# wangqiaoli/geometric_mapping

Hardware: AMD Instinct MI355X
Metric: points/sec full segment+fit, 1M-pt synthetic tunnel frame (higher is better)
Workload: dtype f32; 1 GPU; 1000000-pt synthetic tunnel frame (R=2 m, L=12 m, sigma=0.01), rows resident in HBM; k_regime=fixed-k (~256 neighbours), mode=frames, frames_in_flight=3, GPU_MAX_HW_QUEUES=4, ransac_model=cylinder, H=1024, tau=0.03 (extension), parallelism=framesx1

## Files before the change

### geometric_mapping_amd/csrc/gm_device.hpp

```cpp
#pragma once

#include <hip/hip_runtime.h>
#include <stdint.h>

#include "../../include/gm_hip.h"

namespace gm {

constexpr int kWave = 64;

struct ScanState {
    unsigned long long *status;
    uint32_t *ticket;
    uint32_t epoch;
    const uint32_t *frame_ptr;
};

__device__ __forceinline__ uint32_t scan_epoch(const ScanState &st)
{
    return st.frame_ptr ? 0x20000000u + (((*st.frame_ptr) * 32u + st.epoch) & 0x1FFFFFFFu) : st.epoch;
}

#ifndef GM_TILE_CLASSES
#define GM_TILE_CLASSES 8
#endif
constexpr int kTileListClasses = GM_TILE_CLASSES;

struct DevCounters {
    uint32_t n_cropped;
    uint32_t n_valid;
    uint32_t n_tiles;
    uint32_t first_drop_enc;
    uint32_t n_voxels;
    uint32_t vox_n;
    uint32_t mm[6];
    uint32_t scratch_total;
    uint32_t pad[5];
    uint32_t n_tiles_c[kTileListClasses][32];
};
static_assert(sizeof(DevCounters) % 8 == 0, "zero-filled in 8-byte words");

struct VoxelParams {
    float inv_leaf;
    int32_t min_b[3];
    int32_t div_b[3];
    int32_t mul1, mul2;
    uint32_t passthrough;
};

struct GridParams {
    float ox, oy, oz;
    float inv_h;
    float inv_hx;
    int32_t nx, ny, nz;
    int32_t xreach;
    float r2;
    float r2_scale;
    float snap;
    int32_t D;
    int16_t reach[5][5];
    float dscale;
    float dband;
    float band;
};

struct VoxCell {
    unsigned long long sx, sy, sz;
    uint32_t cnt, pad;
};
struct VoxDense {
    uint32_t enabled;
    int32_t i_lo;
    int32_t dim;
    float inv_leaf;
    float lo;
    float own_lo, own_hi;
    double scale, inv_scale;
    uint32_t xcd_chunk;
    uint32_t pad_;
};

struct FrameExt {
    float plane[4];
    float cylinder[7];
    uint32_t plane_inliers, cylinder_inliers;
    uint32_t pad;
    double plane_refit[4];
    double cyl_axis_refit[3];
};

struct CylFitWork {
    double c[3], d[3], r;
    double d_hyp[3];
    double last_step;
    uint32_t status, passes;
};

struct FrameOut {
    DevCounters ctr;
    float evals[3];
    float evecs[9];
    double scatter[6];
    VoxelParams vox;
    FrameExt ext;
    gm_cylinder_fit fit;
};


__device__ __forceinline__ int lane_id() { return threadIdx.x & (kWave - 1); }

__device__ __forceinline__ uint64_t lanemask_lt()
{
    return (1ull << lane_id()) - 1ull;
}
// ... 285 lines not shown
```

### geometric_mapping_amd/csrc/k_normals.hip

```cpp
#include <stdlib.h>
#include <string.h>

#include "gm_internal.hpp"

namespace gm {

typedef float v2f __attribute__((ext_vector_type(2)));

__device__ __forceinline__ v2f pk_mul_rn(v2f a, v2f b)
{
    v2f r;
    r.x = __fmul_rn(a.x, b.x);
    r.y = __fmul_rn(a.y, b.y);
    return r;
}
__device__ __forceinline__ v2f pk_add_rn(v2f a, v2f b)
{
    v2f r;
    r.x = __fadd_rn(a.x, b.x);
    r.y = __fadd_rn(a.y, b.y);
    return r;
}

__device__ __forceinline__ v2f pk_within(v2f d2, v2f neg_big, v2f r2_big)
// ... 809 lines not shown
                    split3(uxa * uxa, uxb * uxb, 10); split3(uxa * uya, uxb * uyb, 13); split3(uxa * uza, uxb * uzb, 16);
                    split3(uya * uya, uyb * uyb, 19); split3(uya * uza, uyb * uzb, 22); split3(uza * uza, uzb * uzb, 25);
                }
            }
            wave_lds_fence();
            if (c0 + clen < row_end(r)) seek(r, c0 + clen); else seek(r + 1, r + 1 < 9 ? row_begin(r + 1) : 0u);
#pragma unroll
            for (int gi = 0; gi < kMxGroups; ++gi) {
                if (gi >= ngroups) break;
                const uint32_t mb = __builtin_amdgcn_readlane(sb, r * kMxGroups + gi),
                               me = __builtin_amdgcn_readlane(se, r * kMxGroups + gi);
                uint32_t ob = mb > c0 ? mb - c0 : 0u, oe = me > c0 ? me - c0 : 0u;
                if (ob > clen) ob = clen;
                if (oe > clen) oe = clen;
                ob &= ~7u;
                const int steps = oe > ob ? (int)((oe - ob + 15u) >> 4) : 0;
#if defined(GM_NORMALS_STATS) && !defined(GM_MD_DEBUG)
                if (lane == 0) {
                    atomicAdd(&ctr->pad[0], (uint32_t)(steps * 16) / 2u);
                    atomicAdd(&ctr->pad[1], (oe > ob ? oe - ob : 0u) * 2u);
                    if (gi == 0) { atomicAdd(&ctr->pad[2], clen); atomicAdd(&ctr->pad[3], 1u); }
                }
#endif
                const float gqa = __shfl(q.x, gi * kMxGroupLanes + qsel, kWave), gqb = __shfl(q.y, gi * kMxGroupLanes + qsel, kWave),
                            gqc = __shfl(q.z, gi * kMxGroupLanes + qsel, kWave);
                const v2f qx = {gqa, gqa}, qy = {gqb, gqb}, qz = {gqc, gqc};
                const float *pw = wx + ob + 8u * (uint32_t)half;
                const uint32_t *fa = feat + ((ob >> 3) + (uint32_t)half) * (uint32_t)kMxOctetWords + (uint32_t)qsel * 4u;
                constexpr int W = kMxChunk + kMxPad;
                auto ld4 = [](const float *q4) { return *reinterpret_cast<const float4 *>(q4); };
                float4 x0 = ld4(pw), x1 = ld4(pw + 4), y0 = ld4(pw + W), y1 = ld4(pw + W + 4), z0 = ld4(pw + 2 * W),
                       z1 = ld4(pw + 2 * W + 4);
                for (int it = 0; it < steps; ++it) {
                    const bf16x8 a = *reinterpret_cast<const bf16x8 *>(fa);
                    const v2f dx0 = (v2f){x0.x, x0.y} - qx, dx1 = (v2f){x0.z, x0.w} - qx, dx2 = (v2f){x1.x, x1.y} - qx, dx3 = (v2f){x1.z, x1.w} - qx;
                    const v2f dy0 = (v2f){y0.x, y0.y} - qy, dy1 = (v2f){y0.z, y0.w} - qy, dy2 = (v2f){y1.x, y1.y} - qy, dy3 = (v2f){y1.z, y1.w} - qy;
                    const v2f dz0 = (v2f){z0.x, z0.y} - qz, dz1 = (v2f){z0.z, z0.w} - qz, dz2 = (v2f){z1.x, z1.y} - qz, dz3 = (v2f){z1.z, z1.w} - qz;
                    pw += 16; fa += 2 * kMxOctetWords;
                    x0 = ld4(pw); x1 = ld4(pw + 4); y0 = ld4(pw + W); y1 = ld4(pw + W + 4); z0 = ld4(pw + 2 * W); z1 = ld4(pw + 2 * W + 4);
                    __builtin_amdgcn_sched_barrier(0);
                    auto within2 = [&](const v2f dx, const v2f dy, const v2f dz) -> uint32_t {
                        const v2f d2 = pk_add_rn(pk_add_rn(pk_mul_rn(dx, dx), pk_mul_rn(dy, dy)), pk_mul_rn(dz, dz));
                        const v2f wgt = pk_within(d2, neg_big, r2_big);
                        return pack_hi16(__float_as_uint(wgt.y), __float_as_uint(wgt.x));
                    };
                    union { bf16x8 v; uint32_t u[4]; } b;
                    b.u[0] = within2(dx0, dy0, dz0);
                    b.u[1] = within2(dx1, dy1, dz1);
                    b.u[2] = within2(dx2, dy2, dz2);
                    b.u[3] = within2(dx3, dy3, dz3);
                    acc[gi] = __builtin_amdgcn_mfma_f32_32x32x16_bf16(a, b.v, acc[gi], 0, 0, 0);
                }
            }
        }
        float own[16], got[16];
#pragma unroll
        for (int k = 0; k < 16; ++k) {
            own[k] = half ? acc[1][k] : acc[0][k];
            const float snd = half ? acc[0][k] : acc[1][k];
            got[k] = __shfl_xor(snd, 32, kWave);
        }
        auto frow = [&](int rr) -> double {
            const int k = 4 * (rr >> 3) + (rr & 3), hh = (rr >> 2) & 1;
            return (double)((hh == half) ? own[k] : got[k]);
        };
        double mom[10];
        mom[0] = frow(0);
#pragma unroll
        for (int m = 0; m < 9; ++m) mom[1 + m] = (frow(1 + 3 * m) + frow(2 + 3 * m)) + frow(3 + 3 * m);

        const bool vox_ok = emit_normal(active, q, mom, vd, normals4, counts, qn, stat_t0);
        if (vd.enabled) voxel_sums(vox_ok, q, vd, vox_table);
    }
}

typedef short s4 __attribute__((ext_vector_type(4)));
#ifndef GM_MDCHUNK
#define GM_MDCHUNK 128
#endif
constexpr int kMdChunk = GM_MDCHUNK;
constexpr int kMdSlots = kMdChunk + 24;
constexpr int kMdOctets = kMdSlots / 8;
constexpr int kMdOctetWords = 33 * 4;
constexpr int kMdWaveLdsBytes = (kMdOctets * kMdOctetWords + 16) * 4;

constexpr int kRowX[3] = {1, 4, 8}, kRowY[3] = {2, 5, 9}, kRowZ[3] = {3, 6, 10}, kRowQ[3] = {11, 7, 12};
constexpr int kRowProd0 = 13;
__device__ __forceinline__ uint32_t md_window_of_base(int b)
{
    return b < 3 ? 0u : ((b == 3 || b == 8) ? 4u : (b == 9 ? 8u : (b == 10 ? 12u : 0u)));
}
__device__ __forceinline__ void md_split3(float a, uint32_t out[3])
{
    const uint32_t ah = __float_as_uint(a) & 0xFFFF0000u;
    const float ra = a - __uint_as_float(ah);
    const uint32_t am = __float_as_uint(ra) & 0xFFFF0000u;
    const float sa = ra - __uint_as_float(am);
    out[0] = ah >> 16; out[1] = am >> 16; out[2] = __float_as_uint(sa) >> 16;
}
__device__ __forceinline__ s4 md_tr_read(const unsigned char *p)
{
    return __builtin_amdgcn_ds_read_tr16_b64_v4i16((__attribute__((address_space(3))) s4 *)p);
}

#ifndef GM_NORMALS_PREFETCH
#define GM_NORMALS_PREFETCH 1
#endif
#ifdef GM_NORMALS_TIMELINE
__device__ unsigned long long gm_tl_buf[3 * 65536];
#endif
#ifdef GM_NORMALS_PHASES
__device__ unsigned long long gm_phase_ticks[16];
#define GM_PH_STAMP(var) const unsigned long long var = __builtin_amdgcn_s_memtime()
#define GM_PH_ADD(slot, expr) do { ph_acc[slot] += (uint32_t)(expr); } while (0)
#else
#define GM_PH_STAMP(var) do {} while (0)
#define GM_PH_ADD(slot, expr) do {} while (0)
#endif

template <bool FINE>
__device__ __forceinline__ void normals_tile_mxd(const NormalsArgs &A, unsigned char *lds, const uint2 tile, uint32_t min_candidates,
                                                 unsigned long long stat_entry = 0ull)
{
    const float4 *__restrict__ spts4 = A.spts4;
    const uint32_t *__restrict__ skeys = A.skeys;
    DevCounters *__restrict__ ctr = A.ctr;
    const GridParams &g = A.g;
    const uint2 *__restrict__ row_bounds = A.row_bounds;
    float4 *__restrict__ normals4 = A.normals4;
    int32_t *__restrict__ counts = A.counts;
    const VoxDense &vd = A.vd;
    VoxCell *__restrict__ vox_table = A.vox_table;
    (void)ctr;
    uint32_t *feat = reinterpret_cast<uint32_t *>(lds);
    int lane = lane_id();
    asm volatile("" : "+v"(lane));
    const uint32_t n = ctr->n_cropped;
    const int qsel = lane & 31, half = lane >> 5;
    const int tq = (lane & 15) >> 2, tp = lane & 3, tr0 = 16 * ((lane >> 4) & 1);
    const uint32_t tr_off = md_window_of_base(8 * half + tq) * 16u +
                            (uint32_t)((tr0 + 4 * tp) >> 3) * (uint32_t)(kMdOctetWords * 4) + (uint32_t)((tr0 + 4 * tp) & 7) * 2u;
    const uint32_t mom_off = (uint32_t)qsel * 16u + 8u * (uint32_t)half;
    {
        const uint32_t qs = tile.x, qn = tile.y & 0xFFu, tile_row = tile.y >> 8;
#ifdef GM_NORMALS_TIMELINE
        const unsigned long long stat_t0 = wall_clock64();
#else
        const unsigned long long stat_t0 = 0ull;
#endif
#ifdef GM_NORMALS_PHASES
        uint32_t ph_acc[8] = {0, 0, 0, 0, 0, 0, 0, 0};
#endif
        GM_PH_STAMP(ph_t0);
        const bool active = (uint32_t)lane < qn;
        const uint32_t qidx = qs + (active ? (uint32_t)lane : qn - 1u);
        const float4 q = spts4[qidx];
        const uint32_t kl = skeys[qidx];
        const uint32_t row = tile_row;
        const int cy = (int)(row % (uint32_t)g.ny), cz = (int)(row / (uint32_t)g.ny);
        const int gD = FINE ? g.D : 1;
        const int side = 2 * gD + 1, nrows_all = side * side;
        int nrows = 0;
        struct LaneRow { int gg, reach; uint32_t nrow; bool ok; uint2 rb; };
        auto lane_row = [&](int row0) -> LaneRow {
            nrows = nrows_all - row0 < 32 ? nrows_all - row0 : 32;
            const int k = FINE ? lane : (lane >> 1);
            const int r = row0 + (k >> 1);
            const int a = (r % side) - gD, b = (r / side) - gD;
            const int yy = cy + a, zz = cz + b;
            LaneRow R;
            R.gg = k & 1;
            R.reach = (k >> 1) < nrows ? (FINE ? (int)g.reach[a < 0 ? -a : a][b < 0 ? -b : b] : g.xreach) : 0;
            R.ok = R.reach > 0 && yy >= 0 && yy < g.ny && zz >= 0 && zz < g.nz;
            R.nrow = R.ok ? (uint32_t)(zz * g.ny + yy) : 0u;
            R.rb = R.ok ? row_bounds[R.nrow] : make_uint2(0u, 0u);
            return R;
        };
        const LaneRow lr0 = lane_row(0);
        const int fxl = (int)(kl - row * (uint32_t)g.nx);
        if (__ballot(active && q.x >= vd.own_lo && q.x < vd.own_hi) == 0) {
            if (active) {
                const float nanv = __builtin_nanf("");
                normals4[__float_as_uint(q.w)] = make_float4(nanv, nanv, nanv, nanv);
                if (counts) counts[__float_as_uint(q.w)] = 0;
            }
            return;
        }
        uint32_t sb = 0, se = 0;
        auto win_begin = [&](int r, int gg) -> uint32_t {
            return FINE ? __builtin_amdgcn_readlane(sb, r * kMxGroups + gg) : __builtin_amdgcn_readlane(sb, 2 * (r * kMxGroups + gg));
        };
        auto win_end = [&](int r, int gg) -> uint32_t {
            return FINE ? __builtin_amdgcn_readlane(se, r * kMxGroups + gg) : __builtin_amdgcn_readlane(sb, 2 * (r * kMxGroups + gg) + 1);
        };
        auto find_windows = [&](const LaneRow &R) {
            sb = 0; se = 0;
            const int gg = R.gg, reach = R.reach;
            const int lo_fx = __shfl(fxl, gg * kMxGroupLanes, kWave);
            const int hi_fx = __shfl(fxl, gg * kMxGroupLanes + kMxGroupLanes - 1, kWave);
            uint32_t key_b = 0, key_e = 0, lo1 = 0, hi1 = 0, row_key0 = 0;
            if (R.ok) {
                const uint32_t rbk = R.nrow * (uint32_t)g.nx;
                const int xa = lo_fx > reach ? lo_fx - reach : 0;
                const int xb = hi_fx + reach < g.nx - 1 ? hi_fx + reach : g.nx - 1;
                key_b = rbk + (uint32_t)xa; key_e = rbk + (uint32_t)xb + 1u;
                lo1 = R.rb.x; hi1 = R.rb.y; row_key0 = rbk;
            }
            if (FINE) {
                uint32_t lo2 = lo1, hi2 = hi1;
                while (lo1 < hi1 || lo2 < hi2) {
                    const uint32_t m1 = (lo1 + hi1) >> 1, m2 = (lo2 + hi2) >> 1;
                    const uint32_t k1 = skeys[m1 < n ? m1 : n - 1u], k2 = skeys[m2 < n ? m2 : n - 1u];
                    if (lo1 < hi1) { if (k1 < key_b) lo1 = m1 + 1u; else hi1 = m1; }
                    if (lo2 < hi2) { if (k2 < key_e) lo2 = m2 + 1u; else hi2 = m2; }
                }
                sb = lo1; se = lo2;
            } else {
                const uint32_t key = (lane & 1) ? key_e : key_b;
#ifndef GM_NORMALS_NO_GUIDED_PROBE
                constexpr uint32_t kGuide = 64;
                if (hi1 - lo1 > 8u * kGuide) {
                    const uint32_t xq = key - row_key0;
                    const uint32_t gpos = lo1 + (uint32_t)((float)xq * (float)(hi1 - lo1) / (float)g.nx);
                    const uint32_t pa0 = gpos > lo1 + kGuide ? gpos - kGuide : lo1;
                    const uint32_t pb0 = gpos + kGuide < hi1 ? gpos + kGuide : hi1 - 1u;
                    const uint32_t ka0 = skeys[pa0], kb0 = skeys[pb0];
                    if (ka0 < key) lo1 = pa0 + 1u; else hi1 = pa0;
                    if (pb0 >= lo1 && pb0 < hi1) { if (kb0 < key) lo1 = pb0 + 1u; else hi1 = pb0; }
                }
#endif
                while (lo1 < hi1) {
                    const uint32_t m1 = (lo1 + hi1) >> 1;
                    if (skeys[m1] < key) lo1 = m1 + 1u; else hi1 = m1;
                }
                sb = lo1;
            }
        };
        find_windows(lr0);
        GM_PH_STAMP(ph_t1);
        GM_PH_ADD(0, ph_t1 - ph_t0);
        bool thin = false;
        if (!FINE) {
            uint32_t wl = 0;
#pragma unroll
            for (int r = 0; r < 9; ++r)
                wl += win_end(r, 0) - win_begin(r, 0);
            thin = wl < min_candidates;
        }
        const int mid = (int)(qn >> 1);
        const float inv_snap = 1.0f / g.snap;
        const float ox = rintf(__uint_as_float(__builtin_amdgcn_readlane(__float_as_uint(q.x), mid)) * inv_snap) * g.snap,
                    oy = rintf(__uint_as_float(__builtin_amdgcn_readlane(__float_as_uint(q.y), mid)) * inv_snap) * g.snap,
                    oz = rintf(__uint_as_float(__builtin_amdgcn_readlane(__float_as_uint(q.z), mid)) * inv_snap) * g.snap;
#ifdef GM_MD_DEBUG
        const float band = g.band;
#endif
        const int ngroups = qn > (uint32_t)kMxGroupLanes ? 2 : 1;
        f32x16 acc[kMxGroups];

#pragma unroll
        for (int gi = 0; gi < kMxGroups; ++gi)
#pragma unroll
            for (int k = 0; k < 16; ++k) acc[gi][k] = 0.f;

        bf16x8 qb[kMxGroups][2];
        float gq[kMxGroups][3];
#pragma unroll
        for (int gi = 0; gi < kMxGroups; ++gi) {
            gq[gi][0] = __shfl(q.x, gi * kMxGroupLanes + qsel, kWave);
            gq[gi][1] = __shfl(q.y, gi * kMxGroupLanes + qsel, kWave);
            gq[gi][2] = __shfl(q.z, gi * kMxGroupLanes + qsel, kWave);
            const float vx = gq[gi][0] - ox, vy = gq[gi][1] - oy, vz = gq[gi][2] - oz;
            const float vv = __fadd_rn(__fadd_rn(__fmul_rn(vx, vx), __fmul_rn(vy, vy)), __fmul_rn(vz, vz));
            uint32_t sv[3], sx[3], sy[3], sz[3];
            const float S = g.dscale;
            md_split3(__fsub_rn(g.r2, vv) * S, sv); md_split3(2.0f * S * vx, sx); md_split3(2.0f * S * vy, sy); md_split3(2.0f * S * vz, sz);
            const uint32_t one = __float_as_uint(-S) >> 16;
            const uint32_t lo0[8] = {sv[0], sv[1], sv[2], sx[0], sx[0], sx[1], sx[2], sy[0]};
            const uint32_t lo1[8] = {sy[0], sy[1], sy[2], sz[0], sz[0], sz[1], sz[2], one};
            const uint32_t hi0[8] = {sx[1], sx[0], one, 0u, sy[1], sy[0], 0u, 0u};
            const uint32_t hi1[8] = {sz[1], sz[0], 0u, 0u, 0u, one, 0u, 0u};
            union { bf16x8 v; uint32_t u[4]; } f0, f1;
#pragma unroll
            for (int j = 0; j < 4; ++j) {
                f0.u[j] = half ? (hi0[2 * j] | (hi0[2 * j + 1] << 16)) : (lo0[2 * j] | (lo0[2 * j + 1] << 16));
                f1.u[j] = half ? (hi1[2 * j] | (hi1[2 * j + 1] << 16)) : (lo1[2 * j] | (lo1[2 * j + 1] << 16));
            }
            qb[gi][0] = f0.v; qb[gi][1] = f1.v;
        }
        auto row_begin = [&](int r) -> uint32_t { return win_begin(r, 0); };
        auto row_end = [&](int r) -> uint32_t { return win_end(r, ngroups - 1); };
        if (thin) {
            double tm[10] = {0, 0, 0, 0, 0, 0, 0, 0, 0, 0};
            for (int r = 0; r < 9; ++r) {
                const uint32_t e = row_end(r);
                for (uint32_t i = row_begin(r); i < e; ++i) {
                    const float4 c = spts4[i];
                    const float dx = c.x - q.x, dy = c.y - q.y, dz = c.z - q.z;
                    const float d2 = __fadd_rn(__fadd_rn(__fmul_rn(dx, dx), __fmul_rn(dy, dy)), __fmul_rn(dz, dz));
                    if (d2 < g.r2) {
                        const double ex = dx, ey = dy, ez = dz;
                        tm[0] += 1.0; tm[1] += ex; tm[2] += ey; tm[3] += ez;
                        tm[4] += ex * ex; tm[5] += ex * ey; tm[6] += ex * ez; tm[7] += ey * ey; tm[8] += ey * ez; tm[9] += ez * ez;
                    }
                }
            }
            const bool vox_ok = emit_normal(active, q, tm, vd, normals4, counts, qn, stat_t0);
            if (vd.enabled) voxel_sums(vox_ok, q, vd, vox_table);
            return;
        }
        uint32_t gs = 0, stream_total = 0, nxt_c = 0;
        const int endl = 2 * (ngroups - 1) + 1;
        if (!FINE) {
            const int rl = lane & ~3;
            const uint32_t rb = __shfl(sb, rl, kWave), re = __shfl(sb, rl + endl, kWave);
            const bool rowlane = lane < 36;
            const uint32_t len = rowlane ? re - rb : 0u;
            const uint32_t padded = (len + 7u) & ~7u;
            uint32_t incl = padded;
            incl += (uint32_t)__builtin_amdgcn_update_dpp(0, (int)incl, 0x114 , 0xF, 0xF, true);
            incl += (uint32_t)__builtin_amdgcn_update_dpp(0, (int)incl, 0x118 , 0xF, 0xF, true);
            incl += (uint32_t)__builtin_amdgcn_update_dpp(0, (int)incl, 0x142 , 0xA, 0xF, false);
            incl += (uint32_t)__builtin_amdgcn_update_dpp(0, (int)incl, 0x143 , 0xC, 0xF, false);
            const uint32_t srow = incl - padded;
            const uint32_t s_next = __shfl(incl, 4 * (lane - 40), kWave);
            const uint32_t off_r = __shfl(rb - srow, 4 * (lane - 50), kWave);
            gs = rowlane ? srow + (sb - rb) : ((lane >= 40 && lane < 49) ? s_next : ((lane >= 50 && lane < 59) ? off_r : 0u));
            stream_total = __builtin_amdgcn_readlane(gs, 48);
        }
        GM_PH_STAMP(ph_t2);
        GM_PH_ADD(1, ph_t2 - ph_t1);
        static_assert(kMdChunk == 2 * kWave, "one slot pair per lane and chunk");
        constexpr int kMdPieces = 4;
        int cur_r = 0, row0 = 0;
        uint32_t cur_c = row_begin(0);
        uint32_t n_lo[kMxGroups], n_hi[kMxGroups], n_slots = 0;
        float4 pa = make_float4(0.f, 0.f, 0.f, 0.f), pb = pa;
        uint32_t pidx = qs, pv = 0;
        auto assemble_stream = [&]() {
            n_slots = 0; pv = 0; pidx = qs;
#pragma unroll
            for (int gi = 0; gi < kMxGroups; ++gi) { n_lo[gi] = 0xFFFFFFFFu; n_hi[gi] = 0u; }
            if (nxt_c >= stream_total) return;
            const uint32_t c0 = nxt_c, c1 = nxt_c + (uint32_t)kMdChunk;
            nxt_c = c1;
            n_slots = stream_total - c0 < (uint32_t)kMdChunk ? stream_total - c0 : (uint32_t)kMdChunk;
            const uint32_t sl0 = c0 + 2u * (uint32_t)lane;
            uint32_t r = 0;
#pragma unroll
            for (int k = 0; k < 9; ++k) r += sl0 >= (uint32_t)__builtin_amdgcn_readlane(gs, 40 + k) ? 1u : 0u;
            r = r > 8u ? 8u : r;
            const uint32_t off = __shfl(gs, 50 + (int)r, kWave), lim = __shfl(gs, 4 * (int)r + endl, kWave);
            const bool v0 = sl0 < lim, v1 = sl0 + 1u < lim;
            pidx = v0 ? sl0 + off : qs;
            pv = v0 ? (v1 ? 3u : 1u) : 0u;
            const uint32_t other = __shfl_xor(gs, 1, kWave);
            const uint32_t cb = gs > c0 ? gs : c0, ce = other < c1 ? other : c1;
            const uint64_t m = __ballot((lane & 1) == 0 && lane < 36 && ce > cb);
            const uint32_t cb8 = (cb & ~7u) - c0, ce0 = ce - c0;
#pragma unroll
            for (int gi = 0; gi < kMxGroups; ++gi) {
                if (gi >= ngroups) break;
                const uint64_t mg = m & (gi ? 0x444444444ull : 0x111111111ull);
                if (mg) {
                    n_lo[gi] = __builtin_amdgcn_readlane(cb8, (int)__builtin_ctzll(mg));
                    n_hi[gi] = __builtin_amdgcn_readlane(ce0, 63 - (int)__builtin_clzll(mg));
                }
            }
            pa = spts4[pidx];
            pb = spts4[pidx + (pv >> 1)];
        };
        auto assemble_walk = [&]() {
            n_slots = 0; pv = 0; pidx = qs;
#pragma unroll
            for (int gi = 0; gi < kMxGroups; ++gi) { n_lo[gi] = 0xFFFFFFFFu; n_hi[gi] = 0u; }
            int pieces = 0;
            for (;;) {
                if (cur_r >= nrows) {
                    if (!FINE || row0 + 32 >= nrows_all) break;
                    row0 += 32;
                    find_windows(lane_row(row0));
                    cur_r = 0; cur_c = row_begin(0);
                    continue;
                }
                const uint32_t e = row_end(cur_r);
                if (cur_c >= e) {
                    ++cur_r;
                    if (cur_r < nrows) cur_c = row_begin(cur_r);
                    continue;
                }
                const uint32_t len = e - cur_c, room = (uint32_t)kMdChunk - n_slots;
                const uint32_t take = len < room ? len : room;
#pragma unroll
                for (int gi = 0; gi < kMxGroups; ++gi) {
                    if (gi >= ngroups) break;
                    const uint32_t mb = win_begin(cur_r, gi), me = win_end(cur_r, gi);
                    uint32_t ob = mb > cur_c ? mb - cur_c : 0u, oe = me > cur_c ? me - cur_c : 0u;
                    if (ob > take) ob = take;
                    if (oe > take) oe = take;
                    if (oe > ob) {
                        const uint32_t l = n_slots + (ob & ~7u), h = n_slots + oe;
                        n_lo[gi] = l < n_lo[gi] ? l : n_lo[gi];
                        n_hi[gi] = h > n_hi[gi] ? h : n_hi[gi];
                    }
                }
                {
                    const uint32_t i = 2u * (uint32_t)lane;
                    const bool in = i >= n_slots && i < n_slots + take;
                    pidx = in ? cur_c + (i - n_slots) : pidx;
                    pv = in ? (i + 1u < n_slots + take ? 3u : 1u) : pv;
                }
                n_slots += (take + 7u) & ~7u;
                cur_c += take;
                ++pieces;
                if (n_slots >= (uint32_t)kMdChunk || pieces == kMdPieces) break;
            }
            if (n_slots) {
                pa = spts4[pidx];
                pb = spts4[pidx + (pv >> 1)];
            }
        };
        auto assemble = [&]() { if (FINE) assemble_walk(); else assemble_stream(); };
        assemble();
        while (n_slots) {
            uint32_t c_lo[kMxGroups], c_hi[kMxGroups];
#pragma unroll
            for (int gi = 0; gi < kMxGroups; ++gi) { c_lo[gi] = n_lo[gi]; c_hi[gi] = n_hi[gi]; }
#ifdef GM_NORMALS_STATS
            const uint32_t c_slots = n_slots;
#endif
            wave_lds_fence();
            GM_PH_STAMP(ph_c0);
#ifdef GM_NORMALS_PHASES
            asm volatile("s_waitcnt vmcnt(0)" ::: "memory");
            GM_PH_STAMP(ph_c1);
            GM_PH_ADD(2, ph_c1 - ph_c0);
#endif
            {
                const uint32_t i = 2u * (uint32_t)lane;
                const uint32_t oct = i >> 3;
                uint32_t *fo = feat + oct * (uint32_t)kMdOctetWords + ((i & 7u) >> 1);
                auto st = [&](int frow, uint32_t v) { fo[frow * 4] = v; };
                if (pv & 1u) {
                    const bool vb = (pv & 2u) != 0u;
                    const float4 ca = pa, cb = pb;
                    const float uxa = ca.x - ox, uya = ca.y - oy, uza = ca.z - oz;
                    const float uxb = vb ? cb.x - ox : 0.f, uyb = vb ? cb.y - oy : 0.f, uzb = vb ? cb.z - oz : 0.f;
                    auto split3 = [&](float a, float b, int rh, int rm, int rl) {
                        const uint32_t ah = __float_as_uint(a) & 0xFFFF0000u, bh = __float_as_uint(b) & 0xFFFF0000u;
                        st(rh, pack_hi16(bh, ah));
                        const float ra = a - __uint_as_float(ah), rb = b - __uint_as_float(bh);
                        const uint32_t am = __float_as_uint(ra) & 0xFFFF0000u, bm = __float_as_uint(rb) & 0xFFFF0000u;
                        st(rm, pack_hi16(bm, am));
                        const float sa = ra - __uint_as_float(am), sb2 = rb - __uint_as_float(bm);
                        st(rl, pack_hi16(__float_as_uint(sb2), __float_as_uint(sa)));
                    };
                    auto prod3 = [&](float a, float b, int k) { split3(a, b, kRowProd0 + 3 * k, kRowProd0 + 3 * k + 1, kRowProd0 + 3 * k + 2); };
                    st(0, 0x3F803F80u);
                    split3(uxa, uxb, kRowX[0], kRowX[1], kRowX[2]); split3(uya, uyb, kRowY[0], kRowY[1], kRowY[2]);
                    split3(uza, uzb, kRowZ[0], kRowZ[1], kRowZ[2]);
                    const float xxa = uxa * uxa, yya = uya * uya, zza = uza * uza, xxb = uxb * uxb, yyb = uyb * uyb, zzb = uzb * uzb;
                    prod3(xxa, xxb, 0); prod3(uxa * uya, uxb * uyb, 1); prod3(uxa * uza, uxb * uzb, 2);
                    prod3(yya, yyb, 3); prod3(uya * uza, uyb * uzb, 4); prod3(zza, zzb, 5);
                    split3(__fadd_rn(__fadd_rn(xxa, yya), zza), vb ? __fadd_rn(__fadd_rn(xxb, yyb), zzb) : 0x1p100f, kRowQ[0], kRowQ[1], kRowQ[2]);
                    *reinterpret_cast<uint2 *>(feat + oct * (uint32_t)kMdOctetWords + 31u * 4u + (i & 7u)) = make_uint2(pidx, pidx + 1u);
                } else {
                    st(kRowQ[0], 0x71807180u);
                }
                if (lane < (kMdSlots - kMdChunk) / 2)
                    feat[((uint32_t)kMdChunk / 8u + ((uint32_t)lane >> 2)) * (uint32_t)kMdOctetWords + ((uint32_t)lane & 3u) + (uint32_t)kRowQ[0] * 4u] = 0x71807180u;
            }
            wave_lds_fence();
#ifdef GM_PH_ASSEMBLE
            GM_PH_STAMP(ph_ca);
#endif
#if GM_NORMALS_PREFETCH
            assemble();
#endif
            GM_PH_STAMP(ph_c2);
#ifdef GM_NORMALS_PHASES
#ifdef GM_PH_ASSEMBLE
            GM_PH_ADD(2, ph_c2 - ph_ca);
            GM_PH_ADD(3, ph_ca - ph_c1);
#else
            GM_PH_ADD(3, ph_c2 - ph_c1);
#endif
#endif
#pragma unroll
            for (int gi = 0; gi < kMxGroups; ++gi) {
                if (gi >= ngroups) break;
                const uint32_t ob8 = c_lo[gi], oe = c_hi[gi];
#if defined(GM_NORMALS_STATS) && !defined(GM_MD_DEBUG)
                if (lane == 0) {
                    atomicAdd(&ctr->pad[0], (oe > ob8 ? ((oe - ob8 + 31u) >> 5) * 32u : 0u) / 2u);
                    atomicAdd(&ctr->pad[1], (oe > ob8 ? oe - ob8 : 0u) * 2u);
                    if (gi == 0) { atomicAdd(&ctr->pad[2], c_slots); atomicAdd(&ctr->pad[3], 1u); }
                }
#endif
                const int nblk = oe > ob8 ? (int)((oe - ob8 + 31u) >> 5) : 0;
                const unsigned char *fbytes = reinterpret_cast<const unsigned char *>(feat);
                uint32_t p = ob8;
                for (int it = 0; it < nblk; ++it, p += 32u) {
                    const unsigned char *blk = fbytes + (p >> 3) * (uint32_t)(kMdOctetWords * 4);
                    const unsigned char *ta = blk + tr_off;
                    union { bf16x8 v; s4 h[2]; } a0, a1;
                    a0.h[0] = md_tr_read(ta); a0.h[1] = md_tr_read(ta + 16);
                    a1.h[0] = md_tr_read(ta + 32); a1.h[1] = md_tr_read(ta + 48);
                    const unsigned char *ma = blk + mom_off;
                    union { bf16x8 v; uint2 q2[2]; } m0, m1;
                    m0.q2[0] = *reinterpret_cast<const uint2 *>(ma);
                    m0.q2[1] = *reinterpret_cast<const uint2 *>(ma + kMdOctetWords * 4);
                    m1.q2[0] = *reinterpret_cast<const uint2 *>(ma + 2 * kMdOctetWords * 4);
                    m1.q2[1] = *reinterpret_cast<const uint2 *>(ma + 3 * kMdOctetWords * 4);
                    f32x16 d1;
#pragma unroll
                    for (int k = 0; k < 16; ++k) d1[k] = 0.f;
                    d1 = __builtin_amdgcn_mfma_f32_32x32x16_bf16(a0.v, qb[gi][0], d1, 0, 0, 0);
                    d1 = __builtin_amdgcn_mfma_f32_32x32x16_bf16(a1.v, qb[gi][1], d1, 0, 0, 0);
                    uint32_t pw[8];
                    float amin = 3.0e38f;
#pragma unroll
                    for (int k = 0; k < 8; ++k) amin = fminf(fminf(fabsf(d1[2 * k]), fabsf(d1[2 * k + 1])), amin);
#pragma unroll
                    for (int k = 0; k < 8; ++k)
                        asm("v_cvt_pk_bf16_f32 %0, %1, %2 clamp" : "=v"(pw[k]) : "v"(d1[2 * k]), "v"(d1[2 * k + 1]), "v"(amin));
#ifdef GM_MD_DEBUG
                    {
                        const float vx = gq[gi][0] - ox, vy = gq[gi][1] - oy, vz = gq[gi][2] - oz;
#pragma unroll
                        for (int k = 0; k < 16; ++k) {
                            const uint32_t rk = (uint32_t)((k & 3) + 8 * (k >> 2) + 4 * half);
                            if (p + rk < oe) {
                                const float4 c = spts4[feat[((p + rk) >> 3) * (uint32_t)kMdOctetWords + 31u * 4u + ((p + rk) & 7u)]];
                                const float dx = c.x - gq[gi][0], dy = c.y - gq[gi][1], dz = c.z - gq[gi][2];
                                const float d2 = __fadd_rn(__fadd_rn(__fmul_rn(dx, dx), __fmul_rn(dy, dy)), __fmul_rn(dz, dz));
                                const float d1k = g.r2 - d1[k] / g.dscale;
                                const float err = fabsf(d1k - d2) / g.r2;
                                if (d2 < 4.0f * g.r2) {
                                    atomicMax(&ctr->pad[1], __float_as_uint(err));
                                    if (err > 1e-5f) atomicAdd(&ctr->pad[2], 1u);
                                    if (fabsf(d1k - d2) > band) {
                                        atomicAdd(&ctr->pad[0], 1u);
                                        atomicMax(&ctr->pad[3], (uint32_t)(sqrtf(vx * vx + vy * vy + vz * vz) / sqrtf(g.r2) * 1000.f));
                                        const float ux = c.x - ox, uy = c.y - oy, uz = c.z - oz;
                                        atomicMax(&ctr->pad[4], (uint32_t)(sqrtf(ux * ux + uy * uy + uz * uz) / sqrtf(g.r2) * 1000.f));
                                    }
                                }
                            }
                        }
                    }
#endif
                    if (__ballot(amin < g.dband)) {
                        uint32_t gqi = (uint32_t)(gi * kMxGroupLanes + qsel);
                        gqi = qs + (gqi < qn ? gqi : qn - 1u);
                        asm volatile("" : "+v"(gqi));
                        const float4 gqv = spts4[gqi];
#pragma unroll
                        for (int k = 0; k < 16; ++k) {
                            const uint32_t rk = (uint32_t)((k & 3) + 8 * (k >> 2) + 4 * half);
                            const bool need = fabsf(d1[k]) < g.dband;
                            if (__ballot(need)) {
                                if (need) {
                                    const float4 c = spts4[feat[((p + rk) >> 3) * (uint32_t)kMdOctetWords + 31u * 4u + ((p + rk) & 7u)]];
                                    const float dx = c.x - gqv.x, dy = c.y - gqv.y, dz = c.z - gqv.z;
                                    const float d2 = __fadd_rn(__fadd_rn(__fmul_rn(dx, dx), __fmul_rn(dy, dy)), __fmul_rn(dz, dz));
                                    const uint32_t wk = (d2 < g.r2 ? 1u : 0u) * 0x3F80u;
                                    pw[k >> 1] = (k & 1) ? ((pw[k >> 1] & 0x0000FFFFu) | (wk << 16)) : ((pw[k >> 1] & 0xFFFF0000u) | wk);
                                }
                            }
                        }
                    }
                    union { bf16x8 v; uint32_t u[4]; } b0, b1;
#pragma unroll
                    for (int k = 0; k < 4; ++k) { b0.u[k] = pw[k]; b1.u[k] = pw[4 + k]; }
                    acc[gi] = __builtin_amdgcn_mfma_f32_32x32x16_bf16(m0.v, b0.v, acc[gi], 0, 0, 0);
                    acc[gi] = __builtin_amdgcn_mfma_f32_32x32x16_bf16(m1.v, b1.v, acc[gi], 0, 0, 0);
                }
            }
#if !GM_NORMALS_PREFETCH
            assemble();
#endif
            GM_PH_STAMP(ph_c3);
            GM_PH_ADD(4, ph_c3 - ph_c2);
        }
        GM_PH_STAMP(ph_t3);
        int lane_e = lane_id();
        asm volatile("" : "+v"(lane_e));
        const int half_e = lane_e >> 5;
        const bool active_e = (uint32_t)lane_e < qn;
        float own[16], got[16];
#pragma unroll
        for (int k = 0; k < 16; ++k) {
            own[k] = half_e ? acc[1][k] : acc[0][k];
            const float snd = half_e ? acc[0][k] : acc[1][k];
            got[k] = __shfl_xor(snd, 32, kWave);
        }
        auto frow = [&](int rr) -> double {
            const int k = 4 * (rr >> 3) + (rr & 3), hh = (rr >> 2) & 1;
            return (double)((hh == half_e) ? own[k] : got[k]);
        };
        double mom[10];
        mom[0] = frow(0);
        mom[1] = (frow(kRowX[0]) + frow(kRowX[1])) + frow(kRowX[2]);
        mom[2] = (frow(kRowY[0]) + frow(kRowY[1])) + frow(kRowY[2]);
        mom[3] = (frow(kRowZ[0]) + frow(kRowZ[1])) + frow(kRowZ[2]);
#pragma unroll
        for (int m = 0; m < 6; ++m) mom[4 + m] = (frow(kRowProd0 + 3 * m) + frow(kRowProd0 + 3 * m + 1)) + frow(kRowProd0 + 3 * m + 2);

        uint32_t qidx_e = qs + (active_e ? (uint32_t)lane_e : qn - 1u);
        asm volatile("" : "+v"(qidx_e));
        const float4 qe = spts4[qidx_e];
        const bool vox_ok = emit_normal(active_e, qe, mom, vd, normals4, counts, qn, stat_t0, stat_entry);
        if (vd.enabled) voxel_sums(vox_ok, qe, vd, vox_table);
        GM_PH_STAMP(ph_t4);
        GM_PH_ADD(5, ph_t4 - ph_t3);
        GM_PH_ADD(6, ph_t4 - ph_t0);
        GM_PH_ADD(7, 1);
#ifdef GM_NORMALS_PHASES
        if (lane < 8) {
            uint32_t v = 0;
#pragma unroll
            for (int k = 0; k < 8; ++k) v = lane == k ? ph_acc[k] : v;
            atomicAdd(&gm_phase_ticks[lane], (unsigned long long)v);
        }
#endif
    }
}

constexpr int kWaveLdsBytes = (kMxWaveLdsBytes + 15) / 16 * 16;

struct TileList {
    uint32_t n;
    uint32_t pre[kTileClasses];
};
__device__ __forceinline__ TileList tile_list(const NormalsArgs &A)
{
    TileList L;
    uint32_t run = 0;
#pragma unroll
    for (int c = 0; c < kTileClasses; ++c) {
        uint32_t k = A.ctr->n_tiles_c[c][0];
        const uint32_t cap = c + 1 < kTileClasses ? A.tile_seg : A.tiles_cap;
        if (k > cap) k = cap;
        L.pre[c] = run;
        run += k;
    }
    L.n = run;
    return L;
}
__device__ __forceinline__ uint2 tile_at(const NormalsArgs &A, const TileList &L, uint32_t v)
{
    uint32_t c = 0, first = 0;
#pragma unroll
    for (int k = 1; k < kTileClasses; ++k)
        if (v >= L.pre[k]) { c = (uint32_t)k; first = L.pre[k]; }
    return A.tiles[(size_t)c * A.tile_seg + (v - first)];
}

__device__ __forceinline__ uint32_t normals_wave_id(const NormalsArgs &A, uint32_t ntiles)
{
    uint32_t vblock = blockIdx.x;
    const uint32_t nblk = (ntiles + kNrWaves - 1) / kNrWaves;
    if (gridDim.x >= nblk && A.vd.xcd_chunk) {
        if (blockIdx.x >= nblk) return 0xFFFFFFFFu;
        const uint32_t cb = A.vd.xcd_chunk, full = nblk / (8u * cb) * (8u * cb);
        if (blockIdx.x < full) {
            const uint32_t xcd = blockIdx.x % 8u, slot = blockIdx.x / 8u;
            vblock = ((slot / cb) * 8u + xcd) * cb + slot % cb;
        }
    }
    return (uint32_t)__builtin_amdgcn_readfirstlane((int)(vblock * kNrWaves + threadIdx.x / kWave));
}

__global__ __launch_bounds__(kNrThreads, GM_MX_WAVES) void k_normals_m(NormalsArgs A, uint32_t mx_min_candidates)
{
    __shared__ __attribute__((aligned(16))) unsigned char lds[kNrWaves][kWaveLdsBytes];
    const TileList L = tile_list(A);
    const uint32_t ntiles = L.n;
    const uint32_t wave_id = normals_wave_id(A, ntiles), n_waves = gridDim.x * kNrWaves;
    for (uint32_t t = wave_id; t < ntiles; t += n_waves)
        normals_tile_mx(A, lds[threadIdx.x / kWave], tile_at(A, L, t), mx_min_candidates);
}

template <bool FINE>
__global__ __launch_bounds__(kNrThreads, GM_MX_WAVES) void k_normals(NormalsArgs A, uint32_t mx_min_candidates)
{
    __shared__ __attribute__((aligned(16))) unsigned char lds[kNrWaves][(kMdWaveLdsBytes + 15) / 16 * 16];
#ifdef GM_NORMALS_TIMELINE
    unsigned long long stat_entry;
    asm volatile("s_memrealtime %0\n\ts_waitcnt lgkmcnt(0)" : "=s"(stat_entry) : : "memory");
#else
    const unsigned long long stat_entry = 0ull;
#endif
    const TileList L = tile_list(A);
    const uint32_t ntiles = L.n;
    const uint32_t wave_id = normals_wave_id(A, ntiles), n_waves = gridDim.x * kNrWaves;
    if (wave_id >= ntiles) return;
    const int wv = __builtin_amdgcn_readfirstlane((int)(threadIdx.x / kWave));
    {
        uint4 *z = reinterpret_cast<uint4 *>(lds[wv]);
        for (int i = lane_id(); i < kMdWaveLdsBytes / 16; i += kWave) z[i] = make_uint4(0u, 0u, 0u, 0u);
    }
#ifdef GM_NORMALS_TIMELINE
    const uint2 tile_tl = tile_at(A, L, wave_id);
    unsigned long long stat_tile;
    asm volatile("s_memrealtime %0\n\ts_waitcnt lgkmcnt(0)" : "=s"(stat_tile) : "v"(tile_tl.x) : "memory");
    normals_tile_mxd<FINE>(A, lds[wv], tile_tl, mx_min_candidates, stat_entry);
    if (wave_id < 65536u && lane_id() == 0) {
        gm_tl_buf[3 * wave_id + 0] = stat_entry;
        gm_tl_buf[3 * wave_id + 1] = stat_tile;
        gm_tl_buf[3 * wave_id + 2] = (unsigned long long)wall_clock64();
    }
#else
    normals_tile_mxd<FINE>(A, lds[wv], tile_at(A, L, wave_id), mx_min_candidates, stat_entry);
#endif
#ifndef GM_NORMALS_NO_LOOP
    if (ntiles > n_waves && wave_id != 0xFFFFFFFFu)
        for (uint32_t t = wave_id + n_waves; t < ntiles; t += n_waves)
            normals_tile_mxd<FINE>(A, lds[wv], tile_at(A, L, t), mx_min_candidates);
#endif
}

__global__ __launch_bounds__(kNrThreads) void k_normals_valu(NormalsArgs A)
{
    __shared__ __attribute__((aligned(16))) unsigned char lds[kNrWaves][(kValuWaveLdsBytes + 15) / 16 * 16];
    const TileList L = tile_list(A);
    const uint32_t ntiles = L.n;
    const uint32_t wave_id = normals_wave_id(A, ntiles), n_waves = gridDim.x * kNrWaves;
    for (uint32_t t = wave_id; t < ntiles; t += n_waves) normals_tile_valu(A, lds[threadIdx.x / kWave], tile_at(A, L, t));
}

int cell_key_bits(const GridParams &g)
{
    const uint64_t ncell = (uint64_t)g.nx * g.ny * g.nz;
    int bits = 1;
    while ((1ull << bits) < ncell) ++bits;
    return bits;
}

static double inv_below(uint32_t d) { return nextafter(1.0 / (double)(d ? d : 1u), 0.0); }

uint32_t max_tiles(uint32_t n_cap, const GridParams &g)
{
    const uint64_t span = (uint64_t)kTileSpan * (uint64_t)(g.xreach - 1);
    const uint64_t groups = (uint64_t)g.ny * (uint64_t)g.nz * ((uint64_t)g.nx / (span + 1) + 1);
    const uint64_t extra = (groups < n_cap ? groups : n_cap) + n_cap / kTileQ;
    return (uint32_t)(n_cap / kTileQ + extra + 1);
}

void launch_grid_and_normals(const GridParams &g, const VoxDense &vd, Slot &sl, uint32_t n_cap, bool keep_counts,
                             bool scratch_cleared, hipStream_t s)
{
    if (n_cap == 0) return;
    const int where = launch_radix_sort(sl.keys_a, sl.vals_a, sl.keys_b, sl.vals_b, &sl.ctr->n_cropped, n_cap, cell_key_bits(g),
                                        sl, scratch_cleared, s, sl.crop4, sl.spts4);
    uint32_t *skeys = where ? sl.keys_b : sl.keys_a;
    sl.skeys = skeys;
    if (!scratch_cleared) hipMemsetAsync(sl.row_bounds, 0, sizeof(uint2) * (size_t)g.ny * (size_t)g.nz, s);
    {
        ScanState st = next_scan(sl);
        st.status = sl.tile_rec;
        st.ticket = sl.sort.ticket + 1;
        static const char *to = getenv("GM_TILE_ORDER");
        const uint32_t single_class = to ? (to[0] == 'p' ? 1u : 0u) : (sl.pipelined ? 1u : 0u);
        hipLaunchKernelGGL(k_rows_and_tiles, dim3(tile_cutter_blocks(n_cap)), dim3(kTbThreads), 0, s, (const uint32_t *)skeys, sl.ctr,
                           (uint32_t)g.nx, (uint32_t)(kTileSpan * (g.xreach - 1)), inv_below((uint32_t)g.nx),
                           inv_below((uint32_t)(kTileSpan * (g.xreach - 1)) + 1u), sl.row_bounds, (uint32_t)g.ny * (uint32_t)g.nz, sl.tiles,
                           sl.tiles_cap, sl.tile_seg, st, single_class);
    }
    const uint32_t mt = max_tiles(n_cap, g);
    uint32_t nb = (mt + kNrWaves - 1) / kNrWaves;
    {
        const uint32_t usual = (n_cap / 32u + kNrWaves) / kNrWaves;
        if (nb > usual) nb = usual < 64u ? 64u : usual;
    }
    {
        static const char *e = getenv("GM_NORMALS_BLOCKS");
        const uint32_t cap = e ? (uint32_t)atoi(e) : 65536u;
        if (nb > cap) nb = cap;
    }
    static const char *xc = getenv("GM_NORMALS_XCD");
    VoxDense vdx = vd;
    vdx.xcd_chunk = xc ? (uint32_t)atoi(xc) : 32u;
    NormalsArgs na;
    na.spts4 = sl.spts4; na.skeys = skeys; na.tiles = sl.tiles; na.ctr = sl.ctr; na.g = g; na.tiles_cap = sl.tiles_cap; na.tile_seg = sl.tile_seg;
    na.row_bounds = sl.row_bounds; na.normals4 = sl.normals4; na.counts = keep_counts ? sl.counts : (int32_t *)nullptr;
    na.vd = vdx; na.vox_table = sl.vox_table;
    static const char *impl = getenv("GM_NORMALS_IMPL");
    const uint32_t mx_min = !impl ? (uint32_t)kMxMinCandidates : (impl[0] == 'v' ? 0xFFFFFFFFu : (impl[0] == 'm' ? 0u : (uint32_t)kMxMinCandidates));
    if (!sl.capturing) hipEventRecord(sl.ev_k0, s);
    const bool dist_on_mx = !(impl && strchr(impl, '0'));
    if (mx_min == 0xFFFFFFFFu) hipLaunchKernelGGL(k_normals_valu, dim3(nb), dim3(kNrThreads), 0, s, na);
    else if (dist_on_mx) {
        if (g.D > 1) hipLaunchKernelGGL(k_normals<true>, dim3(nb), dim3(kNrThreads), 0, s, na, mx_min);
        else hipLaunchKernelGGL(k_normals<false>, dim3(nb), dim3(kNrThreads), 0, s, na, mx_min);
    }
    else hipLaunchKernelGGL(k_normals_m, dim3(nb), dim3(kNrThreads), 0, s, na, mx_min);
    if (!sl.capturing) hipEventRecord(sl.ev_k1, s);
}

}

#ifdef GM_NORMALS_STATS
extern "C" int gm_debug_counters(gm_ctx *ctx, uint32_t slot, uint32_t *out)
{
    hipDeviceSynchronize();
    gm::DevCounters c;
    const int rc = (int)hipMemcpy(&c, ctx->slots[slot].ctr, sizeof(c), hipMemcpyDeviceToHost);
    memcpy(out, &c, 18 * sizeof(uint32_t));
    out[2] = 0;
    for (int k = 0; k < gm::kTileListClasses; ++k) out[2] += c.n_tiles_c[k][0];
    return rc;
}
#endif

#ifdef GM_NORMALS_TIMELINE
extern "C" int gm_debug_timeline(unsigned long long *out, uint32_t n)
{
    hipDeviceSynchronize();
    if (n > 65536u) n = 65536u;
    return (int)hipMemcpyFromSymbol(out, HIP_SYMBOL(gm::gm_tl_buf), sizeof(unsigned long long) * 3 * (size_t)n);
}
#endif

#ifdef GM_NORMALS_PHASES
extern "C" int gm_debug_phases(unsigned long long *out16)
{
    hipDeviceSynchronize();
    int rc = (int)hipMemcpyFromSymbol(out16, HIP_SYMBOL(gm::gm_phase_ticks), sizeof(unsigned long long) * 16);
    unsigned long long z[16] = {};
    if (rc == 0) rc = (int)hipMemcpyToSymbol(HIP_SYMBOL(gm::gm_phase_ticks), z, sizeof(z));
    return rc;
}
#endif

#ifdef GM_SORT_TIMELINE
extern "C" int gm_debug_cutter_timeline(unsigned long long *out)
{
    hipDeviceSynchronize();
    return (int)hipMemcpyFromSymbol(out, HIP_SYMBOL(gm::gm_cut_tl), sizeof(unsigned long long) * 512 * 8);
}
#endif
```

Before: 4.731 billion points/s.

## Defer near-boundary neighbour candidates to an exact FP32 recheck list

Adds a DEFER variant of the MFMA normals tile for the coarse grid. Candidates whose bf16 distance lies inside an uncertainty band are masked out of the MFMA moment accumulation and recorded in a small per-wave LDS list. After accumulation they are re-tested in exact FP32 and added to the moments on the VALU. If the list overflows, the whole tile is recomputed on the old path. This aims to replace the previous costly band handling with a cheap deferred fixup, at the cost of extra LDS, per-candidate ballots, and a redo when the list overflows. It also swaps a divide for a bit-trick reciprocal of snap and uses ds_bpermute for the xor shuffles.

```diff
diff --git a/geometric_mapping_amd/csrc/gm_device.hpp b/geometric_mapping_amd/csrc/gm_device.hpp
--- a/geometric_mapping_amd/csrc/gm_device.hpp
+++ b/geometric_mapping_amd/csrc/gm_device.hpp
@@ -29,7 +29,7 @@
 struct DevCounters {
     uint32_t n_cropped;
     uint32_t n_valid;
-    uint32_t n_tiles;
+    uint32_t n_band_overflows;
     uint32_t first_drop_enc;
     uint32_t n_voxels;
     uint32_t vox_n;
diff --git a/geometric_mapping_amd/csrc/k_normals.hip b/geometric_mapping_amd/csrc/k_normals.hip
--- a/geometric_mapping_amd/csrc/k_normals.hip
+++ b/geometric_mapping_amd/csrc/k_normals.hip
@@ -915,7 +915,9 @@
 constexpr int kMdSlots = kMdChunk + 24;
 constexpr int kMdOctets = kMdSlots / 8;
 constexpr int kMdOctetWords = 33 * 4;
-constexpr int kMdWaveLdsBytes = (kMdOctets * kMdOctetWords + 16) * 4;
+constexpr int kMdListCap = 32;
+constexpr int kMdListWord = kMdOctets * kMdOctetWords;
+constexpr int kMdWaveLdsBytes = (kMdListWord + kMdListCap) * 4;
 
 constexpr int kRowX[3] = {1, 4, 8}, kRowY[3] = {2, 5, 9}, kRowZ[3] = {3, 6, 10}, kRowQ[3] = {11, 7, 12};
 constexpr int kRowProd0 = 13;
@@ -951,10 +953,16 @@
 #define GM_PH_ADD(slot, expr) do {} while (0)
 #endif
 
-template <bool FINE>
-__device__ __forceinline__ void normals_tile_mxd(const NormalsArgs &A, unsigned char *lds, const uint2 tile, uint32_t min_candidates,
+__device__ __forceinline__ int lane_xor(int v, int lane, int m)
+{
+    return __builtin_amdgcn_ds_bpermute((lane ^ m) << 2, v);
+}
+
+template <bool FINE, bool DEFER = false>
+__device__ __forceinline__ bool normals_tile_mxd(const NormalsArgs &A, unsigned char *lds, const uint2 tile, uint32_t min_candidates,
                                                  unsigned long long stat_entry = 0ull)
 {
+    static_assert(!(FINE && DEFER), "the deferred list is built for the usual grid");
     const float4 *__restrict__ spts4 = A.spts4;
     const uint32_t *__restrict__ skeys = A.skeys;
     DevCounters *__restrict__ ctr = A.ctr;
@@ -1017,7 +1025,7 @@
                 normals4[__float_as_uint(q.w)] = make_float4(nanv, nanv, nanv, nanv);
                 if (counts) counts[__float_as_uint(q.w)] = 0;
             }
-            return;
+            return true;
         }
         uint32_t sb = 0, se = 0;
         auto win_begin = [&](int r, int gg) -> uint32_t {
@@ -1081,7 +1089,7 @@
             thin = wl < min_candidates;
         }
         const int mid = (int)(qn >> 1);
-        const float inv_snap = 1.0f / g.snap;
+        const float inv_snap = __uint_as_float(0x7F000000u - __float_as_uint(g.snap));
         const float ox = rintf(__uint_as_float(__builtin_amdgcn_readlane(__float_as_uint(q.x), mid)) * inv_snap) * g.snap,
                     oy = rintf(__uint_as_float(__builtin_amdgcn_readlane(__float_as_uint(q.y), mid)) * inv_snap) * g.snap,
                     oz = rintf(__uint_as_float(__builtin_amdgcn_readlane(__float_as_uint(q.z), mid)) * inv_snap) * g.snap;
@@ -1140,7 +1148,7 @@
             }
             const bool vox_ok = emit_normal(active, q, tm, vd, normals4, counts, qn, stat_t0);
             if (vd.enabled) voxel_sums(vox_ok, q, vd, vox_table);
-            return;
+            return true;
         }
         uint32_t gs = 0, stream_total = 0, nxt_c = 0;
         const int endl = 2 * (ngroups - 1) + 1;
@@ -1187,7 +1195,7 @@
             const bool v0 = sl0 < lim, v1 = sl0 + 1u < lim;
             pidx = v0 ? sl0 + off : qs;
             pv = v0 ? (v1 ? 3u : 1u) : 0u;
-            const uint32_t other = __shfl_xor(gs, 1, kWave);
+            const uint32_t other = (uint32_t)lane_xor((int)gs, lane, 1);
             const uint32_t cb = gs > c0 ? gs : c0, ce = other < c1 ? other : c1;
             const uint64_t m = __ballot((lane & 1) == 0 && lane < 36 && ce > cb);
             const uint32_t cb8 = (cb & ~7u) - c0, ce0 = ce - c0;
@@ -1254,6 +1262,7 @@
             }
         };
         auto assemble = [&]() { if (FINE) assemble_walk(); else assemble_stream(); };
+        uint32_t n_list = 0;
         assemble();
         while (n_slots) {
             uint32_t c_lo[kMxGroups], c_hi[kMxGroups];
@@ -1319,6 +1328,66 @@
             GM_PH_ADD(3, ph_c2 - ph_c1);
 #endif
 #endif
+            if constexpr (DEFER) {
+                const uint32_t lo = ngroups > 1 ? (c_lo[0] < c_lo[1] ? c_lo[0] : c_lo[1]) : c_lo[0];
+                const uint32_t hi = ngroups > 1 ? (c_hi[0] > c_hi[1] ? c_hi[0] : c_hi[1]) : c_hi[0];
+                const unsigned char *fbytes = reinterpret_cast<const unsigned char *>(feat);
+                for (uint32_t p = lo; p < hi; p += 32u) {
+                    const unsigned char *blk = fbytes + (p >> 3) * (uint32_t)(kMdOctetWords * 4);
+                    const unsigned char *ta = blk + tr_off;
+                    union { bf16x8 v; s4 h[2]; } a0, a1;
+                    a0.h[0] = md_tr_read(ta); a0.h[1] = md_tr_read(ta + 16);
+                    a1.h[0] = md_tr_read(ta + 32); a1.h[1] = md_tr_read(ta + 48);
+                    const unsigned char *ma = blk + mom_off;
+                    union { bf16x8 v; uint2 q2[2]; } m0, m1;
+                    m0.q2[0] = *reinterpret_cast<const uint2 *>(ma);
+                    m0.q2[1] = *reinterpret_cast<const uint2 *>(ma + kMdOctetWords * 4);
+                    m1.q2[0] = *reinterpret_cast<const uint2 *>(ma + 2 * kMdOctetWords * 4);
+                    m1.q2[1] = *reinterpret_cast<const uint2 *>(ma + 3 * kMdOctetWords * 4);
+#pragma unroll
+                    for (int gi = 0; gi < kMxGroups; ++gi) {
+                        if (gi >= ngroups) break;
+                        if (p + 32u <= c_lo[gi] || p >= c_hi[gi]) continue;
+                        f32x16 d1;
+#pragma unroll
+                        for (int k = 0; k < 16; ++k) d1[k] = 0.f;
+                        d1 = __builtin_amdgcn_mfma_f32_32x32x16_bf16(a0.v, qb[gi][0], d1, 0, 0, 0);
+                        d1 = __builtin_amdgcn_mfma_f32_32x32x16_bf16(a1.v, qb[gi][1], d1, 0, 0, 0);
+                        uint32_t pw[8];
+                        float amin = 3.0e38f;
+#pragma unroll
+                        for (int k = 0; k < 8; ++k) amin = fminf(fminf(fabsf(d1[2 * k]), fabsf(d1[2 * k + 1])), amin);
+#pragma unroll
+                        for (int k = 0; k < 8; ++k)
+                            asm("v_cvt_pk_bf16_f32 %0, %1, %2 clamp" : "=v"(pw[k]) : "v"(d1[2 * k]), "v"(d1[2 * k + 1]), "v"(amin));
+                        if (__ballot(amin < g.dband)) {
+#pragma unroll
+                            for (int k = 0; k < 16; ++k) {
+                                const bool need = fabsf(d1[k]) < g.dband;
+                                const uint64_t mk = __ballot(need);
+                                if (mk) {
+                                    if (need) {
+                                        const uint32_t rk = (uint32_t)((k & 3) + 8 * (k >> 2) + 4 * half);
+                                        const uint32_t at = n_list + __builtin_amdgcn_mbcnt_hi((uint32_t)(mk >> 32),
+                                                                     __builtin_amdgcn_mbcnt_lo((uint32_t)mk, 0u));
+                                        pw[k >> 1] &= (k & 1) ? 0x0000FFFFu : 0xFFFF0000u;
+                                        if (at < (uint32_t)kMdListCap) {
+                                            const uint32_t pos = feat[((p + rk) >> 3) * (uint32_t)kMdOctetWords + 31u * 4u + ((p + rk) & 7u)];
+                                            feat[kMdListWord + at] = pos < (1u << 26) - 1u ? (pos << 6) | (uint32_t)(gi * kMxGroupLanes + qsel) : ~0u;
+                                        }
+                                    }
+                                    n_list += (uint32_t)__builtin_popcountll(mk);
+                                }
+                            }
+                        }
+                        union { bf16x8 v; uint32_t u[4]; } b0, b1;
+#pragma unroll
+                        for (int k = 0; k < 4; ++k) { b0.u[k] = pw[k]; b1.u[k] = pw[4 + k]; }
+                        acc[gi] = __builtin_amdgcn_mfma_f32_32x32x16_bf16(m0.v, b0.v, acc[gi], 0, 0, 0);
+                        acc[gi] = __builtin_amdgcn_mfma_f32_32x32x16_bf16(m1.v, b1.v, acc[gi], 0, 0, 0);
+                    }
+                }
+            } else {
 #pragma unroll
             for (int gi = 0; gi < kMxGroups; ++gi) {
                 if (gi >= ngroups) break;
@@ -1410,6 +1479,7 @@
                     acc[gi] = __builtin_amdgcn_mfma_f32_32x32x16_bf16(m1.v, b1.v, acc[gi], 0, 0, 0);
                 }
             }
+            }
 #if !GM_NORMALS_PREFETCH
             assemble();
 #endif
@@ -1421,12 +1491,25 @@
         asm volatile("" : "+v"(lane_e));
         const int half_e = lane_e >> 5;
         const bool active_e = (uint32_t)lane_e < qn;
+        uint32_t ent = 0;
+        if constexpr (DEFER) {
+            wave_lds_fence();
+            bool ovf = n_list > (uint32_t)kMdListCap;
+            if (!ovf && n_list) {
+                ent = (uint32_t)lane_e < n_list ? feat[kMdListWord + lane_e] : 0u;
+                ovf = __ballot(ent == ~0u) != 0ull;
+            }
+            if (ovf) {
+                if (lane_e == 0) atomicAdd(&ctr->n_band_overflows, 1u);
+                return false;
+            }
+        }
         float own[16], got[16];
 #pragma unroll
         for (int k = 0; k < 16; ++k) {
             own[k] = half_e ? acc[1][k] : acc[0][k];
             const float snd = half_e ? acc[0][k] : acc[1][k];
-            got[k] = __shfl_xor(snd, 32, kWave);
+            got[k] = __int_as_float(lane_xor(__float_as_int(snd), lane_e, 32));
         }
         auto frow = [&](int rr) -> double {
             const int k = 4 * (rr >> 3) + (rr & 3), hh = (rr >> 2) & 1;
@@ -1443,6 +1526,28 @@
         uint32_t qidx_e = qs + (active_e ? (uint32_t)lane_e : qn - 1u);
         asm volatile("" : "+v"(qidx_e));
         const float4 qe = spts4[qidx_e];
+        if constexpr (DEFER) {
+            if (n_list) {
+                const bool has = (uint32_t)lane_e < n_list;
+                const uint32_t qid = ent & 63u;
+                const float4 c = spts4[has ? ent >> 6 : qs];
+                const float qx = __shfl(qe.x, (int)qid, kWave), qy = __shfl(qe.y, (int)qid, kWave), qz = __shfl(qe.z, (int)qid, kWave);
+                const float dx = c.x - qx, dy = c.y - qy, dz = c.z - qz;
+                const float d2 = __fadd_rn(__fadd_rn(__fmul_rn(dx, dx), __fmul_rn(dy, dy)), __fmul_rn(dz, dz));
+                const float ux = c.x - ox, uy = c.y - oy, uz = c.z - oz;
+                auto lane_f = [](float v, int j) { return __uint_as_float(__builtin_amdgcn_readlane(__float_as_uint(v), j)); };
+                uint64_t in = __ballot(has && d2 < g.r2);
+                while (in) {
+                    const int j = __builtin_ctzll(in);
+                    in &= in - 1ull;
+                    const double ex = lane_f(ux, j), ey = lane_f(uy, j), ez = lane_f(uz, j);
+                    if (lane_e == __builtin_amdgcn_readlane((int)qid, j)) {
+                        mom[0] += 1.0; mom[1] += ex; mom[2] += ey; mom[3] += ez;
+                        mom[4] += ex * ex; mom[5] += ex * ey; mom[6] += ex * ez; mom[7] += ey * ey; mom[8] += ey * ez; mom[9] += ez * ez;
+                    }
+                }
+            }
+        }
         const bool vox_ok = emit_normal(active_e, qe, mom, vd, normals4, counts, qn, stat_t0, stat_entry);
         if (vd.enabled) voxel_sums(vox_ok, qe, vd, vox_table);
         GM_PH_STAMP(ph_t4);
@@ -1458,6 +1563,7 @@
         }
 #endif
     }
+    return true;
 }
 
 constexpr int kWaveLdsBytes = (kMxWaveLdsBytes + 15) / 16 * 16;
@@ -1515,7 +1621,7 @@
         normals_tile_mx(A, lds[threadIdx.x / kWave], tile_at(A, L, t), mx_min_candidates);
 }
 
-template <bool FINE>
+template <bool FINE, bool DEFER>
 __global__ __launch_bounds__(kNrThreads, GM_MX_WAVES) void k_normals(NormalsArgs A, uint32_t mx_min_candidates)
 {
     __shared__ __attribute__((aligned(16))) unsigned char lds[kNrWaves][(kMdWaveLdsBytes + 15) / 16 * 16];
@@ -1534,23 +1640,28 @@
         uint4 *z = reinterpret_cast<uint4 *>(lds[wv]);
         for (int i = lane_id(); i < kMdWaveLdsBytes / 16; i += kWave) z[i] = make_uint4(0u, 0u, 0u, 0u);
     }
+    auto tile = [&](const uint2 t, unsigned long long se) {
+        if (!normals_tile_mxd<FINE, DEFER>(A, lds[wv], t, mx_min_candidates, se)) {
+            if constexpr (DEFER) normals_tile_mxd<false, false>(A, lds[wv], t, mx_min_candidates, se);
+        }
+    };
 #ifdef GM_NORMALS_TIMELINE
     const uint2 tile_tl = tile_at(A, L, wave_id);
     unsigned long long stat_tile;
     asm volatile("s_memrealtime %0\n\ts_waitcnt lgkmcnt(0)" : "=s"(stat_tile) : "v"(tile_tl.x) : "memory");
-    normals_tile_mxd<FINE>(A, lds[wv], tile_tl, mx_min_candidates, stat_entry);
+    tile(tile_tl, stat_entry);
     if (wave_id < 65536u && lane_id() == 0) {
         gm_tl_buf[3 * wave_id + 0] = stat_entry;
         gm_tl_buf[3 * wave_id + 1] = stat_tile;
         gm_tl_buf[3 * wave_id + 2] = (unsigned long long)wall_clock64();
     }
 #else
-    normals_tile_mxd<FINE>(A, lds[wv], tile_at(A, L, wave_id), mx_min_candidates, stat_entry);
+    tile(tile_at(A, L, wave_id), stat_entry);
 #endif
 #ifndef GM_NORMALS_NO_LOOP
     if (ntiles > n_waves && wave_id != 0xFFFFFFFFu)
         for (uint32_t t = wave_id + n_waves; t < ntiles; t += n_waves)
-            normals_tile_mxd<FINE>(A, lds[wv], tile_at(A, L, t), mx_min_candidates);
+            tile(tile_at(A, L, t), 0ull);
 #endif
 }
 
@@ -1625,8 +1736,11 @@
     const bool dist_on_mx = !(impl && strchr(impl, '0'));
     if (mx_min == 0xFFFFFFFFu) hipLaunchKernelGGL(k_normals_valu, dim3(nb), dim3(kNrThreads), 0, s, na);
     else if (dist_on_mx) {
-        if (g.D > 1) hipLaunchKernelGGL(k_normals<true>, dim3(nb), dim3(kNrThreads), 0, s, na, mx_min);
-        else hipLaunchKernelGGL(k_normals<false>, dim3(nb), dim3(kNrThreads), 0, s, na, mx_min);
+        static const char *df = getenv("GM_NORMALS_DEFER");
+        const bool defer = !(df && df[0] == '0');
+        if (g.D > 1) hipLaunchKernelGGL((k_normals<true, false>), dim3(nb), dim3(kNrThreads), 0, s, na, mx_min);
+        else if (defer) hipLaunchKernelGGL((k_normals<false, true>), dim3(nb), dim3(kNrThreads), 0, s, na, mx_min);
+        else hipLaunchKernelGGL((k_normals<false, false>), dim3(nb), dim3(kNrThreads), 0, s, na, mx_min);
     }
     else hipLaunchKernelGGL(k_normals_m, dim3(nb), dim3(kNrThreads), 0, s, na, mx_min);
     if (!sl.capturing) hipEventRecord(sl.ev_k1, s);
```

New measurement: 4.686 billion points/s (median of 2 runs). Within noise of the previous version (-1.0%).
